# tensor4all/tensor4all-rs

Hardware: AMD Instinct MI355X
Metric: TCI2 full-sweep GF/s (d=30, chi=256 fp64) (higher is better)
Workload: dtype f64

## Files before the change

include/t4a_gpu.h:

```cpp
#ifndef T4A_GPU_H
#define T4A_GPU_H

#include <stddef.h>
#include <stdint.h>

#ifdef __cplusplus
extern "C" {
#endif
#if defined(__GNUC__)
#pragma GCC visibility push(default)
#endif

typedef int32_t t4a_gpu_status;
#define T4A_GPU_SUCCESS 0
#define T4A_GPU_NULL_POINTER (-1)
#define T4A_GPU_INVALID_ARGUMENT (-2)
#define T4A_GPU_BUFFER_TOO_SMALL (-5)
#define T4A_GPU_INTERNAL_ERROR (-6)
#define T4A_GPU_NOT_IMPLEMENTED (-7)
#define T4A_GPU_NAN_ENCOUNTERED (-8)
#define T4A_GPU_SINGULAR_MATRIX (-9)
#define T4A_GPU_NO_DEVICE (-10)
#define T4A_GPU_KERNEL_TIMEOUT (-11)
#define T4A_GPU_CALLBACK_ERROR (-12)
// ... 522 lines not shown
                                                     size_t* added);
t4a_gpu_status t4a_gpu_aci_problem_find_global_pivots(t4a_gpu_aci_problem* h, uint64_t seed, size_t* count, size_t* out);
t4a_gpu_status t4a_gpu_aci_problem_solution(t4a_gpu_aci_problem* h, t4a_gpu_tt** out);
t4a_gpu_status t4a_gpu_aci_problem_frame(t4a_gpu_aci_problem* h, int32_t right, size_t input, size_t site, size_t* rows,
                                         size_t* cols, double* out);
t4a_gpu_status t4a_gpu_aci_problem_errors(const t4a_gpu_aci_problem* h, double* pivot_errors, double* pivot_scales);

t4a_gpu_status t4a_gpu_treeaci_local_update_f64(size_t n_inputs, const size_t* bond_dims, const double* const* row_frames,
                                                const double* const* col_frames, size_t row_count, size_t col_count, int32_t op_kind,
                                                t4a_gpu_aci_op_fn op, void* user, size_t max_bond_dim, double tolerance,
                                                int32_t scale_tolerance, int32_t left_orthogonal, size_t* rank, size_t* row_indices,
                                                size_t* col_indices, double* pivot_errors, size_t* n_pivot_errors, double* left,
                                                double* right, double* sampled_scale, double* local_values);

t4a_gpu_status t4a_gpu_tci2_last_sweep_shapes(const t4a_gpu_tci2* h, size_t* out);
#define T4A_GPU_PROFILE_SLOTS 16
t4a_gpu_status t4a_gpu_tci2_profile_enable(t4a_gpu_tci2* h, int32_t enable);
t4a_gpu_status t4a_gpu_tci2_profile_reset(t4a_gpu_tci2* h);
t4a_gpu_status t4a_gpu_tci2_profile_get(const t4a_gpu_tci2* h, double* out );
t4a_gpu_status t4a_gpu_tci2_profile_variants(const t4a_gpu_tci2* h, double* out , size_t cap_rows, size_t* n_rows);

t4a_gpu_status t4a_gpu_tci2_chain_stats(const t4a_gpu_tci2* h, uint64_t* out );
t4a_gpu_status t4a_gpu_tci2_chain_stats_ext(const t4a_gpu_tci2* h, uint64_t* out );
t4a_gpu_status t4a_gpu_tci2_fill_stats(const t4a_gpu_tci2* h, uint64_t* out );
t4a_gpu_status t4a_gpu_tci2_rook_stats(const t4a_gpu_tci2* h, uint64_t* out );
t4a_gpu_status t4a_gpu_tci2_optimize_group(t4a_gpu_tci2* const* handles, size_t n_handles, const t4a_gpu_tci2_options* options,
                                           int32_t final_sweep1site);
t4a_gpu_status t4a_gpu_tci2_fill_site_tensors_group(t4a_gpu_tci2* const* handles, size_t n_handles);
t4a_gpu_status t4a_gpu_tci2_set_chain(t4a_gpu_tci2* h, int32_t enable, int32_t verify);
t4a_gpu_status t4a_gpu_tci2_set_callback_threads(t4a_gpu_tci2* h, size_t n_threads);
t4a_gpu_status t4a_gpu_tci2_small_stats(const t4a_gpu_tci2* h, uint64_t* out );

t4a_gpu_status t4a_gpu_fn_eval(int32_t fid, int32_t n_acc, const double* params, const uint64_t* weights,
                               const size_t* local_dims, size_t n_sites, const size_t* idx, size_t n_pts,
                               double* out);

#if defined(__GNUC__)
#pragma GCC visibility pop
#endif
#ifdef __cplusplus
}
#endif
#endif
```

tensor4all-rs_amd/csrc/capi.hip:

```cpp
#include "stdrng.hpp"
#include "smallrng.hpp"
#include <memory>
#include <initializer_list>
#include <mutex>

#include "patching.hpp"
#include "tci2.hpp"
#include "tree.hpp"
#include "quantics.hpp"
#include "tensorops.hpp"
#include "dense.hpp"
#include "aci.hpp"
#include "globalsearch.hpp"
#include "mpo.hpp"
#include "contraction.hpp"
#include "quanticstransform.hpp"
#include "tt_canonical.hpp"

struct t4a_gpu_tci2 {
    t4a::Tci2 impl;
    explicit t4a_gpu_tci2(const std::vector<size_t>& d) : impl(d) {}
};

struct t4a_gpu_treetci {
// ... 1065 lines not shown
            out[5 * i + 0] = (double)kv.first;
            for (int j = 0; j < 4; ++j) out[5 * i + 1 + j] = kv.second[j];
            ++i;
        }
    });
}


t4a_gpu_status t4a_gpu_tci2_chain_stats(const t4a_gpu_tci2* h, uint64_t* out)
{
    return guarded([&] {
        T4A_REQUIRE_PTR(h);
        T4A_REQUIRE_PTR(out);
        for (int k = 0; k < 5; ++k) out[k] = h->impl.chain_stats[k];
    });
}

t4a_gpu_status t4a_gpu_tci2_chain_stats_ext(const t4a_gpu_tci2* h, uint64_t* out)
{
    return guarded([&] {
        T4A_REQUIRE_PTR(h);
        T4A_REQUIRE_PTR(out);
        for (int k = 0; k < 4; ++k) out[k] = h->impl.chain_stats_ext[k];
    });
}

t4a_gpu_status t4a_gpu_tci2_rook_stats(const t4a_gpu_tci2* h, uint64_t* out)
{
    return guarded([&] {
        T4A_REQUIRE_PTR(h);
        T4A_REQUIRE_PTR(out);
        const RookWork& w = h->impl.rook_work();
        out[0] = w.n_device_searches;
        out[1] = w.n_device_visits;
        out[2] = w.n_host_searches;
        out[3] = w.n_host_syncs;
    });
}

t4a_gpu_status t4a_gpu_tci2_fill_stats(const t4a_gpu_tci2* h, uint64_t* out)
{
    return guarded([&] {
        T4A_REQUIRE_PTR(h);
        T4A_REQUIRE_PTR(out);
        for (int k = 0; k < 3; ++k) out[k] = h->impl.fill_stats()[k];
    });
// ... 2912 lines not shown
```

tensor4all-rs_amd/csrc/kernels.hpp:

```cpp
#pragma once

#include <hip/hip_runtime.h>

#include <cstddef>
#include <cstdint>

#include "../../include/t4a_testfunctions.h"

namespace t4a {

struct RrluWorkspace;

struct RrluPlan {
    int W = 1;
    int T = 256;
    int cpw = 0;
    int Mld = 0;
    size_t lds_bytes = 0;
};

RrluPlan rrlu_make_plan(int M, int N, int num_cus);

struct RrluArgs {
    const double* A;
// ... 239 lines not shown
    const int* prev_colperm;
    unsigned prev_token;
    unsigned long long* dbg;
    int defer_host_writes;
};
struct ChainWalkArgs {
    char* blocks;
    size_t block_bytes, off_piv, off_rp, off_cp, off_ts;
    double* pi;
    int n_bonds;
    int max_steps;
    double rel_tol, abs_tol;
    double* factors;
    size_t factors_stride;
    unsigned token_base;
    int timed;
    int lean_prep;
    unsigned long long* phase_ticks;
};
void chain_walk_launch(const ChainCommon& c, const FnDevice& fn, const ChainWalkArgs& w, int columns, hipStream_t stream);
void chain_indep_launch(const ChainCommon& c, int n_bonds, hipStream_t stream);
void chain_last_core_launch(const ChainCommon& c, const FnDevice& fn, double* core, int max_entries, hipStream_t stream);
void chain_prep_launch(const ChainCommon& c, const ChainPrepArgs& a, hipStream_t stream);
void chain_pi_launch(const ChainCommon& c, const FnDevice& fn, int b, int n_dep_ub, int n_ind_ub, double* out, hipStream_t stream);

constexpr int CHAIN_GROUP_MAX = 8;
struct ChainGroupSlot {
    ChainCommon c;
    FnDevice fn;
    double* pi;
};
struct ChainPrepGroupArgs {
    ChainPrepArgs a[CHAIN_GROUP_MAX];
};
void chain_indep_group_launch(const ChainGroupSlot* d_slots, int n_handles, int n_bonds, hipStream_t stream);
void chain_prep_group_launch(const ChainGroupSlot* d_slots, const ChainPrepGroupArgs& a, int n_handles, hipStream_t stream);
void chain_pi_group_launch(const ChainGroupSlot* d_slots, int n_handles, int b, int n_dep_ub, int n_ind_ub, hipStream_t stream);

struct GemmDesc {
    int m, n, k;
    const double* A; int lda; long long strideA; int transA;
    const double* B; int ldb; long long strideB; int transB;
    double* C; int ldc; long long strideC;
    double alpha, beta;
    int batch;
    int ksplit = 1;
    double* partial = nullptr;
};
void gemm_launch(const GemmDesc& d, hipStream_t stream);
inline GemmDesc gemm_desc(int m, int n, int k, const double* A, int lda, const double* B, int ldb, double* C, int ldc)
{
    GemmDesc g{};
    g.m = m;
    g.n = n;
    g.k = k;
    g.A = A;
    g.lda = lda;
    g.B = B;
    g.ldb = ldb;
// ... 227 lines not shown
```

tensor4all-rs_amd/csrc/kernels_chain.hip:

```cpp
#include "kernels.hpp"
#include "kernels_rrlu_w1_body.hpp"

namespace t4a {

namespace {

__device__ __forceinline__ const char* chain_kernarg_base()
{
#if defined(__HIP_DEVICE_COMPILE__)
    return (const char*)__builtin_amdgcn_kernarg_segment_ptr();
#else
    return nullptr;
#endif
}

constexpr int CHAIN_T = 1024;
constexpr int WALK_T = 1024;
constexpr int CHAIN_HASH = 4096;

__device__ __forceinline__ unsigned chain_hash(unsigned long long c)
{
    c ^= c >> 33;
    c *= 0xff51afd7ed558ccdull;
    c ^= c >> 29;
    return (unsigned)c & (CHAIN_HASH - 1);
}

__device__ __forceinline__ int block_scan_flag(bool flag, int* wave_sums, int* total)
{
    const int lane = threadIdx.x & 63, wave = threadIdx.x >> 6;
    const unsigned long long bal = __ballot(flag);
    const int before = __builtin_popcountll(bal & ((1ull << lane) - 1ull));
    __syncthreads();
    if (lane == 0) wave_sums[wave] = __builtin_popcountll(bal);
    __syncthreads();
    int base = 0, tot = 0;
    for (int w = 0; w < (int)blockDim.x / 64; ++w) {
        const int v = wave_sums[w];
        if (w < wave) base += v;
        tot += v;
    }
    *total = tot;
    return base + before;
}

template <bool PARENT_OUTER>
__device__ int build_side(const uint64_t* __restrict__ pcode, const uint64_t* __restrict__ pacc, int np, int d,
                          const uint64_t* __restrict__ w, int K, int total_w, int w_off, const uint64_t* __restrict__ ecode,
                          const uint64_t* __restrict__ eacc, int ne, uint64_t* __restrict__ ocode, uint64_t* __restrict__ oacc, int ocap,
// ... 240 lines not shown
        if (np >= 1 && np <= c.cap && ne <= c.cap)
            nd = build_side<false>(par_lds ? ws->par_code : c.J.code + (size_t)(b + 1) * cap, par_lds ? ws->par_acc : c.J.acc + (size_t)(b + 1) * cap * K, np, c.ldim[b + 1], c.w, K, c.total,
                                   c.woff[b + 1], xcode, xacc, ne, c.dep_code, c.dep_acc,
                                   c.dep_cap, s_srcpos, n_prev_dep, mapped ? c.rowmap : nullptr, hkeys, wave_sums);
        lda = n_prev_dep * c.ldim[b + 1] + ne;
    }
    stamp(5);
    if (tid == 0) {
        const int ni = c.ind_cnt[b];
        const bool ok = nd > 0 && ni > 0;
        const int M = c.forward ? nd : ni, N = c.forward ? ni : nd;
        dims[0] = ok ? M : 0;
        dims[1] = ok ? N : 0;
        dims[2] = ok ? 0 : 1;
        dims[3] = mapped ? lda : (ok ? nd : 0);
        if (hdims) {
            hdims[0] = ok ? M : 0;
            hdims[1] = ok ? N : 0;
            hdims[2] = ok ? 0 : 1;
        }
    }
}

__global__ void __launch_bounds__(CHAIN_T) chain_prep_kernel(ChainCommon c, ChainPrepArgs p)
{
    const unsigned long long t0 = p.dbg ? wall_clock64() : 0ull;
    chain_prep_body(c, p, p.dbg);
    if (p.dbg && threadIdx.x == 0) p.dbg[6] += wall_clock64() - t0;
}
__global__ void __launch_bounds__(CHAIN_T) chain_prep_group_kernel(const ChainGroupSlot* __restrict__ slots, ChainPrepGroupArgs g)
{
    const ChainPrepArgs* pa = reinterpret_cast<const ChainPrepArgs*>(chain_kernarg_base() + sizeof(const ChainGroupSlot*)) + blockIdx.x;
    (void)g;
    chain_prep_body(slots[blockIdx.x].c, *pa);
}

__device__ __forceinline__ void chain_pi_body(const ChainCommon& c, const FnDevice& fn, int b, double* __restrict__ out)
{
    const int* dm = c.dims + (size_t)b * 4;
    if (dm[2] != 0) return;
    const int K = fn.n_acc;
    const int nd = c.forward ? dm[0] : dm[1], ni = c.forward ? dm[1] : dm[0];
    const int i = blockIdx.x * blockDim.x + threadIdx.x;
    if (blockIdx.x * (int)blockDim.x >= nd) return;
    uint64_t racc[T4A_FN_MAX_ACC] = {0, 0, 0, 0};
    if (i < nd)
        for (int k = 0; k < K; ++k) racc[k] = c.dep_acc[(size_t)i * K + k];
    const uint64_t* ia = c.ind_acc + (size_t)b * c.ind_cap * K;
    for (int j = blockIdx.y; j < ni; j += gridDim.y) {
        if (i < nd) {
            uint64_t acc[T4A_FN_MAX_ACC] = {0, 0, 0, 0};
            for (int k = 0; k < K; ++k) acc[k] = racc[k] + ia[(size_t)j * K + k];
            out[(size_t)j * nd + i] = t4a_fn_value(fn.fid, acc, fn.params);
        }
    }
}
__global__ void __launch_bounds__(256) chain_pi_kernel(ChainCommon c, FnDevice fn, int b, double* __restrict__ out) { chain_pi_body(c, fn, b, out); }
// ... 8 lines not shown
{
    const int K = c.K;
    const size_t cap = (size_t)c.cap;
    const int gtid = (int)(blockIdx.x * blockDim.x + threadIdx.x), gsz = (int)(gridDim.x * blockDim.x);
    const int lane = (int)(threadIdx.x & 63), gwave = gtid >> 6, nwaves = gsz >> 6;
    for (int pf = gwave; pf < 2 * (nb + 1); pf += nwaves) {
        const int site = pf >> 1, fam = pf & 1;
        if ((fam == 0 && site == 0) || (fam == 1 && site == nb)) continue;
        const ChainTab& T = fam == 0 ? c.I : c.J;
        const ChainTab& Mr = fam == 0 ? c.mI : c.mJ;
        const int cnt = __hip_atomic_load(T.cnt + site, __ATOMIC_RELAXED, __HIP_MEMORY_SCOPE_AGENT);
        if (cnt < 0 || cnt > c.cap) continue;
        for (int e = lane; e < cnt * (1 + K); e += 64) {
            if (e < cnt) Mr.code[(size_t)site * cap + e] = T.code[(size_t)site * cap + e];
            else Mr.acc[(size_t)site * cap * K + (e - cnt)] = T.acc[(size_t)site * cap * K + (e - cnt)];
        }
        if (lane == 0) Mr.cnt[site] = cnt;
    }
    if (c.hdims)
        for (int e = gtid; e < nb * 4; e += gsz)
            if ((e & 3) != 3) c.hdims[e] = __hip_atomic_load(c.dims + e, __ATOMIC_RELAXED, __HIP_MEMORY_SCOPE_AGENT);
}

__global__ void __launch_bounds__(256) chain_last_core_kernel(ChainCommon c, FnDevice fn, double* __restrict__ core, int max_entries)
{
    const int site = c.n_sites - 1, K = c.K;
    const size_t cap = (size_t)c.cap;
    const int L = c.I.cnt[site], R = c.J.cnt[site], S = c.ldim[site], woff = c.woff[site];
    if (L < 1 || L > c.cap || R < 1 || R > c.cap || S < 1) return;
    const long long total = (long long)L * S * R;
    if (total > (long long)max_entries) return;
    for (long long e = (long long)blockIdx.x * blockDim.x + threadIdx.x; e < total; e += (long long)gridDim.x * blockDim.x) {
        const int l = (int)(e % L), s_ = (int)((e / L) % S), r = (int)(e / ((long long)L * S));
        uint64_t acc[T4A_FN_MAX_ACC] = {0, 0, 0, 0};
        for (int q = 0; q < K; ++q)
            acc[q] = c.I.acc[((size_t)site * cap + l) * K + q] + c.w[(size_t)q * c.total + woff + s_] + c.J.acc[((size_t)site * cap + r) * K + q];
        core[e] = t4a_fn_value(fn.fid, acc, fn.params);
    }
}

__device__ __forceinline__ void walk_phase_barrier(bool scalar_cache = true)
{
    if (scalar_cache) {
        __syncthreads();
        __builtin_amdgcn_s_dcache_inv();
        asm volatile("s_waitcnt lgkmcnt(0)" ::: "memory");
    } else {
        asm volatile("s_waitcnt lgkmcnt(0)\n\ts_barrier" ::: "memory");
    }
}
__device__ __forceinline__ int walk_div_small(int x, float rd) { return (int)(((float)x + 0.5f) * rd); }
__device__ __forceinline__ int walk_load_i32(const int* p) { return __hip_atomic_load(p, __ATOMIC_RELAXED, __HIP_MEMORY_SCOPE_AGENT); }

template <bool FORWARD>
__device__ __forceinline__ void walk_prep_wave0(const ChainCommon& c, WalkShared* ws, int b, int prev_b, unsigned prev_token, bool do_build, unsigned long long* dbg = nullptr)
{
    const unsigned long long dbg_t0 = dbg ? wall_clock64() : 0ull;
    const int lane = threadIdx.x & 63;
    const int K = c.K;
    const size_t cap = (size_t)c.cap;
    bool poison = false;
    int np = 0;
    if (prev_b >= 0) {
        const int pb = prev_b;
        const int pm = ws->dims[pb * 4], pn = ws->dims[pb * 4 + 1];
        const bool bad = ws->dims[pb * 4 + 2] != 0 || ws->prev_ires[1] != 0 || ws->prev_ires[3] != (int)prev_token || pm <= 0 || pn <= 0;
        const int r = ws->prev_ires[0];
        const int cnt = r > 0 ? r : 1;
        if (bad || cnt > c.cap || cnt > pm || cnt > pn || cnt > WALK_MAX_LIST) {
            poison = true;
        } else {
// ... 263 lines not shown
                    if (tid == 0) a.iresult[3] = (int)a.salt;
                }
            }
            if (tid == 0) {
                ws->prev_ires[0] = npiv >= 0 ? npiv : 0;
                ws->prev_ires[1] = npiv >= 0 ? 0 : 1;
                ws->prev_ires[2] = 0;
                ws->prev_ires[3] = npiv >= 0 ? (int)(w.token_base + (unsigned)k) : 0;
            }
        }
        walk_phase_barrier(!w.lean_prep);
        phase(2);
    }
    for (int e = tid; e < nb * 4; e += (int)blockDim.x) c.dims[e] = ws->dims[e];
    __threadfence();
    __syncthreads();
    chain_mirror_body(c, nb);
    if (w.phase_ticks && tid == 0) {
        for (int i = 0; i < 3; ++i) w.phase_ticks[i] = ph[i];
        w.phase_ticks[3] = wall_clock64() - ph_t0;
    }
}

template <int NC, bool FORWARD, bool FACTORS> void chain_walk_launch_one(const ChainCommon& c, const FnDevice& fn, const ChainWalkArgs& w, hipStream_t stream)
{
    constexpr size_t lds = walk_lds_bytes<NC, FACTORS>();
    static std::once_flag attr_once;
    std::call_once(attr_once, [] {
        (void)hipFuncSetAttribute(reinterpret_cast<const void*>(&chain_walk_kernel<NC, FORWARD, FACTORS>), hipFuncAttributeMaxDynamicSharedMemorySize, (int)lds);
    });
    hipLaunchKernelGGL((chain_walk_kernel<NC, FORWARD, FACTORS>), dim3(1), dim3(WALK_T), lds, stream, c, fn, w);
}

template <int NC> void chain_walk_launch_nc(const ChainCommon& c, const FnDevice& fn, const ChainWalkArgs& w, hipStream_t stream)
{
    if (w.factors) {
        if (c.forward) chain_walk_launch_one<NC, true, true>(c, fn, w, stream);
        else chain_walk_launch_one<NC, false, true>(c, fn, w, stream);
    } else {
        if (c.forward) chain_walk_launch_one<NC, true, false>(c, fn, w, stream);
        else chain_walk_launch_one<NC, false, false>(c, fn, w, stream);
    }
}

}

void chain_indep_launch(const ChainCommon& c, int n_bonds, hipStream_t stream)
{
    hipLaunchKernelGGL(chain_indep_kernel, dim3(n_bonds), dim3(CHAIN_T), 0, stream, c);
}

void chain_prep_launch(const ChainCommon& c, const ChainPrepArgs& a, hipStream_t stream)
{
    hipLaunchKernelGGL(chain_prep_kernel, dim3(1), dim3(CHAIN_T), 0, stream, c, a);
}

void chain_pi_launch(const ChainCommon& c, const FnDevice& fn, int b, int n_dep_ub, int n_ind_ub, double* out, hipStream_t stream)
{
    if (n_dep_ub <= 0 || n_ind_ub <= 0) return;
    const int gy = n_ind_ub < 2048 ? n_ind_ub : 2048;
    hipLaunchKernelGGL(chain_pi_kernel, dim3((n_dep_ub + 255) / 256, gy), dim3(256), 0, stream, c, fn, b, out);
}

void chain_indep_group_launch(const ChainGroupSlot* d_slots, int n_handles, int n_bonds, hipStream_t stream)
{
    hipLaunchKernelGGL(chain_indep_group_kernel, dim3(n_bonds, n_handles), dim3(CHAIN_T), 0, stream, d_slots);
}

void chain_prep_group_launch(const ChainGroupSlot* d_slots, const ChainPrepGroupArgs& a, int n_handles, hipStream_t stream)
{
    hipLaunchKernelGGL(chain_prep_group_kernel, dim3(n_handles), dim3(CHAIN_T), 0, stream, d_slots, a);
}

void chain_pi_group_launch(const ChainGroupSlot* d_slots, int n_handles, int b, int n_dep_ub, int n_ind_ub, hipStream_t stream)
{
    if (n_dep_ub <= 0 || n_ind_ub <= 0 || n_handles <= 0) return;
    const int gy = n_ind_ub < 2048 ? n_ind_ub : 2048;
    hipLaunchKernelGGL(chain_pi_group_kernel, dim3((n_dep_ub + 255) / 256, gy, n_handles), dim3(256), 0, stream, d_slots, b);
}

void chain_walk_launch(const ChainCommon& c, const FnDevice& fn, const ChainWalkArgs& w, int columns, hipStream_t stream)
{
    if (columns <= 8) chain_walk_launch_nc<8>(c, fn, w, stream);
    else if (columns <= 16) chain_walk_launch_nc<16>(c, fn, w, stream);
    else chain_walk_launch_nc<32>(c, fn, w, stream);
}

void chain_last_core_launch(const ChainCommon& c, const FnDevice& fn, double* core, int max_entries, hipStream_t stream)
{
    const int blocks = max_entries > 256 * 64 ? 64 : (max_entries + 255) / 256;
    hipLaunchKernelGGL(chain_last_core_kernel, dim3(blocks > 0 ? blocks : 1), dim3(256), 0, stream, c, fn, core, max_entries);
}

}
// ... 1 lines not shown
```

tensor4all-rs_amd/csrc/tci2.hpp:

```cpp
#pragma once

#include <cstring>
#include <memory>
#include <vector>

#include "engine.hpp"
#include "fnsource.hpp"
#include "matrix_source.hpp"
#include "stdrng.hpp"
#include "pishard.hpp"
#include "rook.hpp"
#include "tt.hpp"

namespace t4a {

struct TCI2Options {
    double tolerance = 1e-8;
    size_t max_iter = 20;
    size_t max_bond_dim = 0;
    int pivot_search = 0;
    bool normalize_error = true;
    size_t verbosity = 0;
    size_t max_nglobal_pivot = 5;
    size_t nsearch = 5;
// ... 99 lines not shown
    bool small_engine_run(OptRun& r);
    void opt_begin(OptRun& r);
    void opt_issue_pending_fill(OptRun& r);
    bool opt_iter_start(OptRun& r, bool defer_launch = false);
    void opt_iter_finish(OptRun& r);
    void opt_end(OptRun& r);
    void sweep2site(bool forward, const TCI2Options& options);
    void sweep1site(bool forward, double rel_tol, double abs_tol, size_t max_bond_dim, bool update_tensors);
    void fill_site_tensors();
    void fill_wait();
    void export_site_tensors_async(double* d_dst, size_t stride, hipStream_t consumer);
    void export_site_shard_async(double* d_dst, size_t stride, hipStream_t consumer);
    void import_site_shard_async(const double* d_src, size_t stride, size_t per_rank, hipStream_t producer);
    void make_canonical(double rel_tol, double abs_tol, size_t max_bond_dim);
    void invalidate_site_tensors();
    void flush_pivot_errors() { pivot_errors.clear(); }
    void mark_sets_changed()
    {
        chain_.tables_valid = false;
        chain_.digits_stale = false;
    }
    std::array<uint64_t, 5> chain_stats{{0, 0, 0, 0, 0}};
    std::array<uint64_t, 4> chain_stats_ext{{0, 0, 0, 0}};
    const uint64_t* fill_stats() const { return fill_.stats; }
    const RookWork& rook_work() const { return rook_work_; }
    bool chain_enabled = true;
    bool chain_verify = false;
    bool chain_event_timing = false;

    std::vector<double> evaluate(const uint32_t* idx, size_t n_pts);
    double sum();
    std::vector<double> site_tensor_host(size_t site, size_t dims3[3]);

    void assign_from_tensor_train(const TensorTrain& tt, const FromTensorTrainOptions& options);

    size_t n_;
    std::vector<size_t> local_dims;
    std::vector<IndexSet> i_set, j_set;
    struct HistEntry {
        std::vector<IndexSet> is, js;
        bool digits_valid = true;
        std::vector<uint64_t> code;
        size_t cap = 0;
        uint64_t serial = 0;
    };
    std::vector<HistEntry> history;
// ... 118 lines not shown
        DevBuf<int> dims;
        PinBuf<int> hdims;
        bool inflight = false;
        bool forward = true;
        bool in_optimize = false;
        long ext_idx = -1;
        size_t chi = 0;
        std::vector<size_t> order;
        std::vector<RrluRoute> plans;
        std::vector<unsigned> tokens;
        bool one_site = false;
        bool one_factors = false;
        double abs_tol = 0.0;
        DevBuf<double> factors, urows;
        size_t factors_stride = 0;
        bool cores_batched = false;
        bool last_core_launched = false, last_core_ok = false;
        DevBuf<unsigned long long> walk_dbg;
        bool walked = false;
        bool prep_dbg = false;
        unsigned walk_token = 1;
        RrluBlock proto;
        bool timed = false, timed_events = false;
        std::vector<hipEvent_t> t0, t1;
        bool prepared = false;
        ChainCommon common;
        std::vector<size_t> dep_ub, ind_ub;
        bool use_extras = false;
        size_t ind_cap = 0, cap_side = 0;
        double tol = 0.0;
        hipStream_t wait_stream = nullptr;
        int group_role = 0;
        hipEvent_t group_ev = nullptr;
        DevBuf<ChainGroupSlot> gslots;
        PinBuf<ChainGroupSlot> hgslots;
    } chain_;
    bool chain_usable(const TCI2Options& options) const;
    ChainTab chain_tab(int family) const;
    ChainTab chain_mirror(int which, int family) const;
    void chain_layout(size_t cap);
    void chain_upload_current();
    void chain_upload_hist(HistEntry& e, int slot);
    uint64_t code_of(const uint32_t* v, size_t first_site, size_t width, bool prefix) const;
    void decode_set(IndexSet& s, const uint64_t* codes, size_t first_site, bool prefix) const;
    void hist_digits(HistEntry& e);
    bool chain_enqueue(bool forward, const TCI2Options& options, long ext_idx, bool in_optimize, bool launch = true);
// ... 27 lines not shown
```

tensor4all-rs_amd/csrc/tci2_chain.hip:

```cpp
#include "tci2.hpp"

#include <algorithm>
#include <atomic>
#include <chrono>
#include <cmath>
#include <cstdlib>

namespace t4a {

namespace {
size_t round_up_sz(size_t v, size_t m) { return (v + m - 1) / m * m; }
std::atomic<int> g_chains_inflight{0};
}
thread_local double g_chain_wait_seconds = 0.0;

bool Tci2::chain_usable(const TCI2Options& options) const
{
    static const bool off = std::getenv("T4A_NO_CHAIN") != nullptr;
    if (off || !chain_enabled || !fn_.builtin() || options.pivot_search != 0) return false;
    long double space = 1.0L;
    for (size_t d : local_dims) space *= (long double)d;
    if (space >= 9.0e18L) return false;
    for (size_t p = 0; p < n_; ++p) {
        if (i_set[p].count == 0 || j_set[p].count == 0) return false;
// ... 469 lines not shown
            chain_walk_launch(c, fn_.dev, w, (int)walk_cols, st);
            ++chain_stats_ext[0];
        }
        static const bool want_prep_dbg = std::getenv("T4A_PREP_DEBUG") != nullptr;
        unsigned long long* prep_dbg = nullptr;
        if (want_prep_dbg && !walk) {
            chain_.walk_dbg.reserve(8);
            T4A_HIP(hipMemsetAsync(chain_.walk_dbg.get(), 0, 8 * sizeof(unsigned long long), st));
            prep_dbg = chain_.walk_dbg.get();
            chain_.prep_dbg = true;
        }
        bool spec_pending = false;
        for (size_t k = 0; !walk && k < nb; ++k) {
            const size_t b = order[k];
            const RrluRoute& pl = plans[b];
            const bool fused = pl.fused;
            const bool spec_here = spec_pending && !fused;
            const RrluBlock blk = block_of(b);
            ChainPrepArgs pa;
            std::memset(&pa, 0, sizeof(pa));
            pa.b = (int)b;
            pa.do_build = 1;
            pa.dbg = prep_dbg;
            pa.defer_host_writes = 0;
            pa.with_rowmap = spec_here ? 1 : 0;
            pa.prev_b = -1;
            if (k > 0) {
                const size_t pb = order[k - 1];
                const RrluBlock pblk = block_of(pb);
                pa.prev_b = (int)pb;
                pa.prev_iresult = pblk.iresult();
                pa.prev_rowperm = pblk.row_perm();
                pa.prev_colperm = pblk.col_perm();
                pa.prev_token = tokens[pb];
            }
            chain_prep_launch(c, pa, st);
            if (!fused && !spec_here) chain_pi_launch(c, fn_.dev, (int)b, (int)dep_ub[b], (int)ind_ub[b], chain_.pi.get(), st);
            XcdSpecArgs sp;
            std::memset(&sp, 0, sizeof(sp));
            spec_pending = false;
            if (solo && k + 1 < nb && pl.on_xcd()) {
                const size_t nx = order[k + 1];
                if (!plans[nx].fused) {
                    const size_t site = forward ? nx : nx + 1;
                    const ChainTab& H = forward ? c.HI : c.HJ;
                    const size_t hsite = forward ? nx + 1 : nx;
                    sp.out = chain_.spec[(k + 1) & 1].get();
// ... 8 lines not shown
                    sp.d = (int)local_dims[site];
                    sp.fn = fn_.dev;
                    spec_pending = true;
                }
            }
            FusedPi fp;
            fp.fn = fn_.dev;
            fp.d_rowacc = c.dep_acc;
            fp.d_colacc = c.ind_acc + b * ind_cap * K;
            fp.host_resident = false;
            const double* A = fused ? nullptr : (spec_here ? chain_.spec[k & 1].get() : chain_.pi.get());
            if (timed_events) T4A_HIP(hipEventRecord(chain_.t0[b], st));
            tokens[b] = eng.chain_rrlu(pl, forward, A, spec_here ? c.rowmap : nullptr, fused ? &fp : nullptr, c.dims + b * 4, chi, chain_.tol,
                                       chain_.one_site ? chain_.abs_tol : 0.0, blk, spec_pending ? &sp : nullptr,
                                       chain_.factors_stride ? chain_.factors.get() + b * chain_.factors_stride : nullptr, chain_.urows.get());
            if (timed_events) T4A_HIP(hipEventRecord(chain_.t1[b], st));
        }
        if (!walk) {
            const size_t pb = order[nb - 1];
            const RrluBlock pblk = block_of(pb);
            ChainPrepArgs pa;
            std::memset(&pa, 0, sizeof(pa));
            pa.do_build = 0;
            pa.defer_host_writes = 0;
            pa.prev_b = (int)pb;
            pa.prev_iresult = pblk.iresult();
            pa.prev_rowperm = pblk.row_perm();
            pa.prev_colperm = pblk.col_perm();
            pa.prev_token = tokens[pb];
            chain_prep_launch(c, pa, st);
        }
        chain_.cores_batched = false;
        if (chain_.one_site && chain_.factors_stride && forward && nb <= (size_t)LUCI_LEFT_CORES_MAX_JOBS) {
            LeftCoreJobs jobs;
            std::memset(&jobs, 0, sizeof(jobs));
            size_t max_rows = 1;
            for (size_t b = 0; b < nb; ++b) {
                const RrluBlock blk = block_of(b);
                const size_t rub = std::max<size_t>(std::min({dep_ub[b], ind_ub[b], chi}), 1);
                DevCore& core = cores[b];
                core.buf.reserve(std::max<size_t>(dep_ub[b] * rub, 1));
                LeftCoreJob& j = jobs.j[b];
                j.lu = chain_.factors.get() + b * chain_.factors_stride;
                j.dims = c.dims + b * 4;
                j.iresult = blk.iresult();
                j.row_perm = blk.row_perm();
                j.core = core.buf.get();
                j.S = (int)local_dims[b];
                j.token = tokens[b];
                max_rows = std::max(max_rows, dep_ub[b]);
            }
            luci_left_cores_batched_launch(jobs, (int)nb, (int)max_rows, st);
            chain_.cores_batched = true;
// ... 89 lines not shown
        auto block_of = [&](Tci2* h, size_t b) {
            RrluBlock k = h->chain_.proto;
            k.dev = h->chain_.blocks.get() + b * k.bytes;
            return k;
        };
        auto prev_of = [&](Tci2* h, size_t pb, ChainPrepArgs& pa) {
            const RrluBlock pblk = block_of(h, pb);
            pa.prev_b = (int)pb;
            pa.prev_iresult = pblk.iresult();
            pa.prev_rowperm = pblk.row_perm();
            pa.prev_colperm = pblk.col_perm();
            pa.prev_token = h->chain_.tokens[pb];
        };
        chain_indep_group_launch(d_slots, (int)nh, (int)nb, st);
        const std::vector<size_t>& order = lead->chain_.order;
        for (size_t k = 0; k < nb; ++k) {
            const size_t b = order[k];
            ChainPrepGroupArgs pg;
            std::memset(&pg, 0, sizeof(pg));
            for (size_t i = 0; i < nh; ++i) {
                ChainPrepArgs& pa = pg.a[i];
                pa.b = (int)b;
                pa.do_build = 1;
                pa.prev_b = -1;
                if (k > 0) prev_of(hs[i], order[k - 1], pa);
            }
            chain_prep_group_launch(d_slots, pg, (int)nh, st);
            chain_pi_group_launch(d_slots, (int)nh, (int)b, gplans[b].kM, gplans[b].kN, st);
            RrluXcdGroupArgs ga;
            std::memset(&ga, 0, sizeof(ga));
            for (int x = 0; x < 8; ++x) ga.p[x].xcc = -1;
            for (size_t i = 0; i < nh; ++i) {
                Tci2* h = hs[i];
                h->chain_.tokens[b] = h->eng.chain_group_args(gplans[b], forward, h->chain_.pi.get(), h->chain_.common.dims + b * 4, h->chain_.chi,
                                                              h->chain_.tol, 0.0, block_of(h, b), (int)i, &ga.p[i], st);
            }
            gplans[b].launch_group(ga, !forward, st);
        }
        {
            ChainPrepGroupArgs pg;
            std::memset(&pg, 0, sizeof(pg));
            for (size_t i = 0; i < nh; ++i) prev_of(hs[i], order[nb - 1], pg.a[i]);
            chain_prep_group_launch(d_slots, pg, (int)nh, st);
        }
        for (Tci2* h : hs)
            T4A_HIP(hipMemcpyAsync(h->chain_.hblocks.get(), h->chain_.blocks.get(), nb * h->chain_.proto.bytes, hipMemcpyDeviceToHost, st));
        T4A_HIP(hipGetLastError());
    } catch (...) {
        (void)hipStreamSynchronize(st);
        if (locked) lead->eng.chain_end();
        for (size_t i = 0; i < nh; ++i) {
            if (counted[i]) g_chains_inflight.fetch_sub(1);
            hs[i]->chain_.prepared = false;
            hs[i]->chain_.tables_valid = false;
            hs[i]->chain_.snap_serial[0] = hs[i]->chain_.snap_serial[1] = ~0ull;
        }
        throw;
    }
    for (Tci2* h : hs) {
        h->chain_.plans = gplans;
        h->chain_.inflight = true;
        h->chain_.wait_stream = st;
        h->chain_.group_role = h == lead ? 1 : 2;
    }
}

// ... 69 lines not shown
        if (hi[1] != 0 || hi[3] != (int)chain_.tokens[b]) {
            failed_k = (long)k;
            failed_timeout = hi[1] != 2;
            break;
        }
        if (hi[2] != 0) {
            failed_k = (long)k;
            break;
        }
    }
    if (failed_k >= 0) {
        static const bool dbg = std::getenv("T4A_CHAIN_DEBUG") != nullptr;
        if (dbg) {
            const size_t b = chain_.order[(size_t)failed_k];
            const int* hd = chain_.hdims.get() + b * 4;
            const int* hi = reinterpret_cast<const int*>(chain_.hblocks.get() + b * proto.bytes + 16);
            const RrluRoute& pl = chain_.plans[b];
            std::fprintf(stderr, "[t4a chain] bond %zu (k = %ld of %zu, %s) did not complete: dims %d x %d poisoned %d lda %d | npiv %d flag %d nan %d token %d (want %u) | plan kind %d %d x %d wg %d RPT %d CPT %d W %d\n",
                         b, failed_k, nb, forward ? "forward" : "backward", hd[0], hd[1], hd[2], hd[3], hi[0], hi[1], hi[2], hi[3], chain_.tokens[b], (int)pl.kind, pl.kM, pl.kN,
                         pl.xcd.wg, pl.xcd.RPT, pl.xcd.CPT, pl.xcd.W);
        }
    }
    const size_t done = failed_k < 0 ? nb : (size_t)failed_k;
    for (size_t k = 0; k < done; ++k) {
        const size_t b = chain_.order[k];
        const int* hd = chain_.hdims.get() + b * 4;
        const char* hb = chain_.hblocks.get() + b * proto.bytes;
        const int* hi = reinterpret_cast<const int*>(hb + 16);
        const size_t M = (size_t)hd[0], N = (size_t)hd[1];
        const int rank = hi[0];
        double last_error, abs_max;
        std::memcpy(&last_error, hb, sizeof(double));
        std::memcpy(&abs_max, hb + 8, sizeof(double));
        const size_t cnt = (size_t)(rank > 0 ? rank : 1);
        if ((size_t)ni.cnt[b + 1] != cnt || (size_t)nj.cnt[b] != cnt)
            throw Error(T4A_GPU_INTERNAL_ERROR, "bond chain: gathered pivot count of bond " + std::to_string(b) + " disagrees with its rank");
        i_set[b + 1].count = cnt;
        j_set[b].count = cnt;
        i_set[b + 1].d.clear();
        j_set[b].d.clear();
        {
            float ms = 0.f;
            if (chain_.timed) {
                unsigned long long ts[2];
                std::memcpy(ts, hb + proto.off_ts, sizeof(ts));
                ms = ts[1] > ts[0] ? (float)((double)(ts[1] - ts[0]) * 1e-5) : 0.f;
                if (chain_.timed_events) T4A_HIP(hipEventElapsedTime(&ms, chain_.t0[b], chain_.t1[b]));
                eng.prof.v[0] += ms;
                eng.prof.v[1] += 1.0;
            }
            eng.rrlu_account(chain_.plans[b], !forward, (int)M, (int)N, rank, chain_.timed, ms, chain_.chi > 0 && (size_t)rank == chain_.chi);
            eng.prof.v[11] += (double)M * (double)N;
        }
        if (abs_max > max_sample_value) max_sample_value = abs_max;
        bond_errors[b] = last_error;
        if (chain_.one_site) {
            std::vector<double> pe((size_t)rank + 1);
            const double* pv = reinterpret_cast<const double*>(hb + proto.off_piv);
            for (int q = 0; q < rank; ++q) pe[(size_t)q] = std::sqrt(pv[q] * pv[q]);
            pe[(size_t)rank] = last_error;
            update_pivot_errors(pe);
        } else {
            last_sweep_shapes[b] = {M, N, (size_t)rank};
        }
    }
    if (done > 0) {
        const ChainTab oi = chain_mirror(chain_.mcur, 0), oj = chain_mirror(chain_.mcur, 1);
        std::vector<char> wi(n_, 0), wj(n_, 0);
        for (size_t k = 0; k < done; ++k) {
// ... 130 lines not shown
```

tensor4all-rs_amd/python/t4a_amd/__init__.py:

```python
import ctypes
import os

import numpy as np

from .functions import (FnSpec, quantics_trig_exp, quantics_osc2d, lorentz, linear_sum,
                        FN_MAX_PARAMS)

_HERE = os.path.dirname(os.path.abspath(__file__))
LIB_PATH = os.environ.get("T4A_GPU_LIB") or os.path.normpath(os.path.join(_HERE, "..", "..", "lib", "libt4a_gpu.so"))

if not os.path.exists(LIB_PATH):
    raise ImportError(f"{LIB_PATH} not found: build it with `python tensor4all-rs_amd/build.py` "
                      "(the MI355X backend has no CPU fallback)")

_lib = ctypes.CDLL(LIB_PATH)

c_size_t = ctypes.c_size_t
c_double = ctypes.c_double
c_int32 = ctypes.c_int32
c_void_p = ctypes.c_void_p

SUCCESS = 0
NULL_POINTER = -1
INVALID_ARGUMENT = -2
# ... 737 lines not shown
        _check(_lib.t4a_gpu_tci2_small_stats(self._h, out))
        return {"completed": int(out[0]), "iterations": int(out[1]), "handed_back": int(out[2]), "not_eligible": int(out[3]),
                "device_us": (out[4] / 100.0, out[5] / 100.0, out[6] / 100.0), "reason": int(out[7]),
                "phase_cycles": dict(zip(("lists", "evaluation", "pivot_steps", "gather", "factors", "fill", "snapshots", "rest"), (int(out[8 + k]) for k in range(8))))}

    def rook_stats(self):
        out = (ctypes.c_uint64 * 4)()
        _check(_lib.t4a_gpu_tci2_rook_stats(self._h, out))
        return {"device_searches": int(out[0]), "device_visits": int(out[1]), "host_searches": int(out[2]), "host_syncs": int(out[3])}

    def fill_stats(self):
        out = (ctypes.c_uint64 * 3)()
        _check(_lib.t4a_gpu_tci2_fill_stats(self._h, out))
        return {"fills": int(out[0]), "graph_replays": int(out[1]), "graph_captures": int(out[2])}

    def chain_stats(self):
        out = np.zeros(5, dtype=np.uint64)
        _check(_lib.t4a_gpu_tci2_chain_stats(self._h, _p(out)))
        ext = np.zeros(4, dtype=np.uint64)
        _check(_lib.t4a_gpu_tci2_chain_stats_ext(self._h, _p(ext)))
        return dict(half_sweeps=int(out[0]), bonds=int(out[1]), fell_back=int(out[2]), not_eligible=int(out[3]),
                    group_half_sweeps=int(out[4]), walked_sweeps=int(ext[0]), one_site_sweeps=int(ext[1]),
                    one_site_not_eligible=int(ext[2]), one_site_fell_back=int(ext[3]))


def optimize_group(tcis, options, final_sweep1site=True):
    o = options.to_c()
    arr = (c_void_p * len(tcis))(*[t._h for t in tcis])
    _check(_lib.t4a_gpu_tci2_optimize_group(arr, c_size_t(len(tcis)), ctypes.byref(o), c_int32(1 if final_sweep1site else 0)))


def fill_site_tensors_group(tcis):
    arr = (c_void_p * len(tcis))(*[t._h for t in tcis])
    _check(_lib.t4a_gpu_tci2_fill_site_tensors_group(arr, c_size_t(len(tcis))))


def crossinterpolate2(f, local_dims, initial_pivots, options):
    options.to_c()
    tci = TensorCI2(local_dims)
    tci.set_function(f)
    tci.crossinterpolate2(initial_pivots, options)
    return tci


def svd_backend(a):
    a = _f(a)
# ... 1212 lines not shown
```

Baseline: 329.6.

## Add lean LDS-staged chain prep kernel and defer host-mirror writes to batched mirror pass

```diff
diff --git a/include/t4a_gpu.h b/include/t4a_gpu.h
--- a/include/t4a_gpu.h
+++ b/include/t4a_gpu.h
@@ -568,6 +568,7 @@
 
 t4a_gpu_status t4a_gpu_tci2_chain_stats(const t4a_gpu_tci2* h, uint64_t* out );
 t4a_gpu_status t4a_gpu_tci2_chain_stats_ext(const t4a_gpu_tci2* h, uint64_t* out );
+t4a_gpu_status t4a_gpu_tci2_chain_handover(const t4a_gpu_tci2* h, size_t* count, double* interval_us, int32_t* steps);
 t4a_gpu_status t4a_gpu_tci2_fill_stats(const t4a_gpu_tci2* h, uint64_t* out );
 t4a_gpu_status t4a_gpu_tci2_rook_stats(const t4a_gpu_tci2* h, uint64_t* out );
 t4a_gpu_status t4a_gpu_tci2_optimize_group(t4a_gpu_tci2* const* handles, size_t n_handles, const t4a_gpu_tci2_options* options,
diff --git a/tensor4all-rs_amd/csrc/capi.hip b/tensor4all-rs_amd/csrc/capi.hip
--- a/tensor4all-rs_amd/csrc/capi.hip
+++ b/tensor4all-rs_amd/csrc/capi.hip
@@ -1111,6 +1111,21 @@
         T4A_REQUIRE_PTR(h);
         T4A_REQUIRE_PTR(out);
         for (int k = 0; k < 4; ++k) out[k] = h->impl.chain_stats_ext[k];
+    });
+}
+
+t4a_gpu_status t4a_gpu_tci2_chain_handover(const t4a_gpu_tci2* h, size_t* count, double* interval_us, int32_t* steps)
+{
+    return guarded([&] {
+        T4A_REQUIRE_PTR(h);
+        T4A_REQUIRE_PTR(count);
+        const auto& v = h->impl.chain_handover();
+        *count = v.size();
+        if (interval_us && steps)
+            for (size_t k = 0; k < v.size(); ++k) {
+                interval_us[k] = v[k][0];
+                steps[k] = (int32_t)v[k][1];
+            }
     });
 }
 
diff --git a/tensor4all-rs_amd/csrc/kernels.hpp b/tensor4all-rs_amd/csrc/kernels.hpp
--- a/tensor4all-rs_amd/csrc/kernels.hpp
+++ b/tensor4all-rs_amd/csrc/kernels.hpp
@@ -285,6 +285,7 @@
 void chain_indep_launch(const ChainCommon& c, int n_bonds, hipStream_t stream);
 void chain_last_core_launch(const ChainCommon& c, const FnDevice& fn, double* core, int max_entries, hipStream_t stream);
 void chain_prep_launch(const ChainCommon& c, const ChainPrepArgs& a, hipStream_t stream);
+void chain_mirror_launch(const ChainCommon& c, int n_bonds, hipStream_t stream);
 void chain_pi_launch(const ChainCommon& c, const FnDevice& fn, int b, int n_dep_ub, int n_ind_ub, double* out, hipStream_t stream);
 
 constexpr int CHAIN_GROUP_MAX = 8;
@@ -298,6 +299,7 @@
 };
 void chain_indep_group_launch(const ChainGroupSlot* d_slots, int n_handles, int n_bonds, hipStream_t stream);
 void chain_prep_group_launch(const ChainGroupSlot* d_slots, const ChainPrepGroupArgs& a, int n_handles, hipStream_t stream);
+void chain_mirror_group_launch(const ChainGroupSlot* d_slots, int n_handles, int n_bonds, hipStream_t stream);
 void chain_pi_group_launch(const ChainGroupSlot* d_slots, int n_handles, int b, int n_dep_ub, int n_ind_ub, hipStream_t stream);
 
 struct GemmDesc {
diff --git a/tensor4all-rs_amd/csrc/kernels_chain.hip b/tensor4all-rs_amd/csrc/kernels_chain.hip
--- a/tensor4all-rs_amd/csrc/kernels_chain.hip
+++ b/tensor4all-rs_amd/csrc/kernels_chain.hip
@@ -1,5 +1,6 @@
 #include "kernels.hpp"
 #include "kernels_rrlu_w1_body.hpp"
+#include <atomic>
 
 namespace t4a {
 
@@ -25,6 +26,11 @@
     c ^= c >> 29;
     return (unsigned)c & (CHAIN_HASH - 1);
 }
+
+__device__ __forceinline__ void chain_lds_barrier() { asm volatile("s_waitcnt lgkmcnt(0)\n\ts_barrier" ::: "memory"); }
+
+__device__ __forceinline__ void chain_touch(uint64_t v) { asm volatile("" ::"v"(v) : "memory"); }
+__device__ __forceinline__ void chain_touch(int v) { asm volatile("" ::"v"(v) : "memory"); }
 
 __device__ __forceinline__ int block_scan_flag(bool flag, int* wave_sums, int* total)
 {
@@ -311,17 +317,262 @@
     }
 }
 
+constexpr int PREP_MAX_W = 2 * CHAIN_T;
+static_assert(CHAIN_MAX_SET <= CHAIN_T, "the lean preparation keeps one table entry (parent, extra, permutation entry) per thread");
+static_assert(CHAIN_T / 64 <= 64, "the wave counts of the compaction are combined by the lanes of one wave");
+struct PrepShared {
+    unsigned long long hkeys[CHAIN_HASH];
+    uint64_t par_code[CHAIN_MAX_SET], par_acc[CHAIN_MAX_SET * T4A_FN_MAX_ACC];
+    uint64_t w[PREP_MAX_W];
+    int srcpos[CHAIN_MAX_SET];
+    int wave_sums[CHAIN_T / 64];
+};
+
+__device__ __forceinline__ void chain_prep_lean_body(const ChainCommon& c, const ChainPrepArgs& p, PrepShared* sh, unsigned long long* dbg)
+{
+    unsigned long long dbg_last = dbg ? wall_clock64() : 0ull;
+    auto stamp = [&](int slot) {
+        if (dbg) {
+            const unsigned long long now = wall_clock64();
+            if (threadIdx.x == 0) dbg[slot] += now - dbg_last;
+            dbg_last = now;
+        }
+    };
+    const int tid = threadIdx.x, lane = tid & 63, wave = tid >> 6;
+    const int K = c.K, capi = c.cap;
+    const size_t cap = (size_t)c.cap;
+    const bool fwd = c.forward != 0, have_prev = p.prev_b >= 0, build = p.do_build != 0;
+    const bool extras = build && c.use_extras != 0;
+    const int pb = have_prev ? p.prev_b : 0, b = build ? p.b : 0;
+    if (capi < 1 || capi > CHAIN_MAX_SET || K < 1 || K > T4A_FN_MAX_ACC) return;
+    const int tcl = tid < capi ? tid : capi - 1;
+    if (extras) {
+#pragma unroll
+        for (int e = 0; e < CHAIN_HASH / CHAIN_T; ++e) sh->hkeys[tid + e * CHAIN_T] = 0ull;
+    }
+
+    const int* const pd = c.dims + (size_t)pb * 4;
+    const int* const irp = have_prev ? p.prev_iresult : c.dims;
+    const int rlim_ = fwd ? c.dep_cap : c.ind_cap, clim_ = fwd ? c.ind_cap : c.dep_cap;
+    const int rlim = have_prev && rlim_ > 1 ? rlim_ : 1, clim = have_prev && clim_ > 1 ? clim_ : 1;
+    const int* const rpp = have_prev ? p.prev_rowperm : c.dims;
+    const int* const cpp = have_prev ? p.prev_colperm : c.dims;
+    const int site = fwd ? b : b + 1;
+    const int hsite = fwd ? b + 1 : b;
+    const ChainTab& H = fwd ? c.HI : c.HJ;
+    const ChainTab& PT = fwd ? c.I : c.J;
+    const int nw = K * c.total;
+    const bool w_lds = nw >= 1 && nw <= PREP_MAX_W;
+    const int nwc = nw < 1 ? 1 : (nw > PREP_MAX_W ? PREP_MAX_W : nw);
+    const int pd0 = pd[0], pd1 = pd[1], pd2 = pd[2];
+    const int ir0 = irp[0], ir1 = irp[1], ir3 = irp[3];
+    const int rp = rpp[tcl < rlim ? tcl : rlim - 1], cp = cpp[tcl < clim ? tcl : clim - 1];
+    const int ni = c.ind_cnt[b], d = c.ldim[site], woff = c.woff[site];
+    const int ne_raw = H.cnt[hsite], np0 = PT.cnt[site];
+    const uint64_t w0 = c.w[tid < nwc ? tid : nwc - 1], w1 = c.w[tid + CHAIN_T < nwc ? tid + CHAIN_T : nwc - 1];
+    const uint64_t xc = H.code[(size_t)hsite * cap + tcl];
+    uint64_t xa[T4A_FN_MAX_ACC], pa[T4A_FN_MAX_ACC];
+#pragma unroll
+    for (int q = 0; q < T4A_FN_MAX_ACC; ++q) xa[q] = H.acc[((size_t)hsite * cap + tcl) * K + (q < K ? q : K - 1)];
+    uint64_t pc = PT.code[(size_t)site * cap + tcl];
+#pragma unroll
+    for (int q = 0; q < T4A_FN_MAX_ACC; ++q) pa[q] = PT.acc[((size_t)site * cap + tcl) * K + (q < K ? q : K - 1)];
+
+    const bool bad = (pd2 != 0) | (ir1 != 0) | (ir3 != (int)p.prev_token) | (pd0 <= 0) | (pd1 <= 0);
+    const int r = ir0;
+    const int cnt = r > 0 ? r : 1;
+    const bool poison = have_prev & (bad | (cnt > capi) | (cnt > pd0) | (cnt > pd1));
+    const int n_prev_dep = (have_prev & !poison) ? (fwd ? pd0 : pd1) : 0;
+
+    const bool gather = have_prev && !poison;
+    chain_touch(rp), chain_touch(cp);
+    const bool mine = gather && tid < cnt;
+    uint64_t rc = 0, cc = 0, ra[T4A_FN_MAX_ACC] = {0, 0, 0, 0}, ca[T4A_FN_MAX_ACC] = {0, 0, 0, 0};
+    int src = 0;
+    if (gather) {
+        const uint64_t* const pind_code = c.ind_code + (size_t)pb * c.ind_cap;
+        const uint64_t* const pind_acc = c.ind_acc + (size_t)pb * c.ind_cap * K;
+        const uint64_t* rcode = fwd ? c.dep_code : pind_code;
+        const uint64_t* racc = fwd ? c.dep_acc : pind_acc;
+        const uint64_t* ccode = fwd ? pind_code : c.dep_code;
+        const uint64_t* cacc = fwd ? pind_acc : c.dep_acc;
+        const int ri = (mine && r > 0) ? rp : 0, ci = (mine && r > 0) ? cp : 0;
+        rc = rcode[ri];
+        cc = ccode[ci];
+#pragma unroll
+        for (int q = 0; q < T4A_FN_MAX_ACC; ++q) {
+            ra[q] = racc[(size_t)ri * K + (q < K ? q : K - 1)];
+            ca[q] = cacc[(size_t)ci * K + (q < K ? q : K - 1)];
+        }
+        src = fwd ? ri : ci;
+    }
+    const unsigned long long xkey = (unsigned long long)(xc / (uint64_t)(d > 0 ? d : 1)) + 1ull;
+    chain_touch(rc), chain_touch(cc), chain_touch(xc), chain_touch(pc), chain_touch(w0), chain_touch(w1);
+#pragma unroll
+    for (int q = 0; q < T4A_FN_MAX_ACC; ++q) chain_touch(ra[q]), chain_touch(ca[q]), chain_touch(xa[q]), chain_touch(pa[q]);
+    if (gather) {
+        pc = fwd ? rc : cc;
+#pragma unroll
+        for (int q = 0; q < T4A_FN_MAX_ACC; ++q) pa[q] = fwd ? ra[q] : ca[q];
+    }
+    const int np = have_prev ? cnt : np0;
+    const int ne = extras ? ne_raw : 0;
+    const bool sides_ok = np >= 1 && np <= capi && ne <= capi;
+    if (build && !poison) {
+        if (sides_ok && tid < np) {
+            sh->par_code[tid] = pc;
+#pragma unroll
+            for (int q = 0; q < T4A_FN_MAX_ACC; ++q)
+                if (q < K) sh->par_acc[(size_t)tid * K + q] = pa[q];
+            sh->srcpos[tid] = src;
+        }
+        if (w_lds) {
+            if (tid < nw) sh->w[tid] = w0;
+            if (tid + CHAIN_T < nw) sh->w[tid + CHAIN_T] = w1;
+        }
+    }
+    if (mine) {
+        const size_t oi = (size_t)(pb + 1) * cap + tid, oj = (size_t)pb * cap + tid;
+        c.I.code[oi] = rc;
+        c.J.code[oj] = cc;
+#pragma unroll
+        for (int q = 0; q < T4A_FN_MAX_ACC; ++q)
+            if (q < K) {
+                c.I.acc[oi * K + q] = ra[q];
+                c.J.acc[oj * K + q] = ca[q];
+            }
+        if (!p.defer_host_writes) {
+            c.mI.code[oi] = rc;
+            c.mJ.code[oj] = cc;
+#pragma unroll
+            for (int q = 0; q < T4A_FN_MAX_ACC; ++q)
+                if (q < K) {
+                    c.mI.acc[oi * K + q] = ra[q];
+                    c.mJ.acc[oj * K + q] = ca[q];
+                }
+        }
+    }
+    if (gather && tid == 0) {
+        c.I.cnt[pb + 1] = cnt;
+        c.J.cnt[pb] = cnt;
+        if (!p.defer_host_writes) {
+            c.mI.cnt[pb + 1] = cnt;
+            c.mJ.cnt[pb] = cnt;
+        }
+    }
+    stamp(4);
+    if (!build) return;
+    int* dims = c.dims + (size_t)b * 4;
+    int* hdims = (c.hdims && !p.defer_host_writes) ? c.hdims + (size_t)b * 4 : nullptr;
+    if (poison) {
+        if (tid == 0) {
+            dims[0] = dims[1] = dims[3] = 0;
+            dims[2] = 1;
+            if (hdims) {
+                hdims[0] = hdims[1] = 0;
+                hdims[2] = 1;
+            }
+        }
+        return;
+    }
+
+    const bool mapped = have_prev && p.with_rowmap;
+    chain_lds_barrier();
+    int nd = -1;
+    const int m0 = np * d;
+    if (sides_ok && m0 <= c.dep_cap) {
+        auto kron = [&](const uint64_t* __restrict__ wsrc) {
+            for (int idx = tid; idx < m0; idx += CHAIN_T) {
+                const int i = fwd ? idx / d : idx % np;
+                const int s = fwd ? idx % d : idx / np;
+                c.dep_code[idx] = (uint64_t)s + (uint64_t)d * sh->par_code[i];
+                for (int k = 0; k < K; ++k) c.dep_acc[(size_t)idx * K + k] = sh->par_acc[(size_t)i * K + k] + wsrc[(size_t)k * c.total + woff + s];
+                if (mapped) c.rowmap[idx] = sh->srcpos[i] * d + s;
+            }
+        };
+        if (w_lds) kron(sh->w);
+        else kron(c.w);
+        if (ne <= 0) {
+            nd = m0;
+        } else {
+            if (tid < np) {
+                const unsigned long long key = (unsigned long long)pc + 1ull;
+                unsigned h = chain_hash(key);
+                for (;;) {
+                    const unsigned long long old = atomicCAS(&sh->hkeys[h], 0ull, key);
+                    if (old == 0ull || old == key) break;
+                    h = (h + 1) & (CHAIN_HASH - 1);
+                }
+            }
+            chain_lds_barrier();
+            bool keep = false;
+            if (tid < ne) {
+                unsigned h = chain_hash(xkey);
+                keep = true;
+                for (;;) {
+                    const unsigned long long v = sh->hkeys[h];
+                    if (v == 0ull) break;
+                    if (v == xkey) {
+                        keep = false;
+                        break;
+                    }
+                    h = (h + 1) & (CHAIN_HASH - 1);
+                }
+            }
+            const unsigned long long bal = __ballot(keep);
+            if (lane == 0) sh->wave_sums[wave] = __builtin_popcountll(bal);
+            chain_lds_barrier();
+            int v = lane < CHAIN_T / 64 ? sh->wave_sums[lane] : 0;
+            int vb = lane < wave ? v : 0;
+#pragma unroll
+            for (int off = 32; off >= 1; off >>= 1) {
+                v += __shfl_xor(v, off);
+                vb += __shfl_xor(vb, off);
+            }
+            const int tot = v;
+            if (m0 + tot <= c.dep_cap) {
+                if (keep) {
+                    const int o = m0 + vb + __builtin_popcountll(bal & ((1ull << lane) - 1ull));
+                    c.dep_code[o] = xc;
+#pragma unroll
+                    for (int k = 0; k < T4A_FN_MAX_ACC; ++k)
+                        if (k < K) c.dep_acc[(size_t)o * K + k] = xa[k];
+                    if (mapped) c.rowmap[o] = n_prev_dep * d + tid;
+                }
+                nd = m0 + tot;
+            }
+        }
+    }
+    stamp(5);
+    if (tid == 0) {
+        const int lda = n_prev_dep * d + ne;
+        const bool ok = nd > 0 && ni > 0;
+        const int M = fwd ? nd : ni, N = fwd ? ni : nd;
+        dims[0] = ok ? M : 0;
+        dims[1] = ok ? N : 0;
+        dims[2] = ok ? 0 : 1;
+        dims[3] = mapped ? lda : (ok ? nd : 0);
+        if (hdims) {
+            hdims[0] = ok ? M : 0;
+            hdims[1] = ok ? N : 0;
+            hdims[2] = ok ? 0 : 1;
+        }
+    }
+}
+
 __global__ void __launch_bounds__(CHAIN_T) chain_prep_kernel(ChainCommon c, ChainPrepArgs p)
 {
+    extern __shared__ __attribute__((aligned(16))) char prep_lds[];
     const unsigned long long t0 = p.dbg ? wall_clock64() : 0ull;
-    chain_prep_body(c, p, p.dbg);
+    chain_prep_lean_body(c, p, reinterpret_cast<PrepShared*>(prep_lds), p.dbg);
     if (p.dbg && threadIdx.x == 0) p.dbg[6] += wall_clock64() - t0;
 }
 __global__ void __launch_bounds__(CHAIN_T) chain_prep_group_kernel(const ChainGroupSlot* __restrict__ slots, ChainPrepGroupArgs g)
 {
+    extern __shared__ __attribute__((aligned(16))) char prep_group_lds[];
     const ChainPrepArgs* pa = reinterpret_cast<const ChainPrepArgs*>(chain_kernarg_base() + sizeof(const ChainGroupSlot*)) + blockIdx.x;
     (void)g;
-    chain_prep_body(slots[blockIdx.x].c, *pa);
+    chain_prep_lean_body(slots[blockIdx.x].c, *pa, reinterpret_cast<PrepShared*>(prep_group_lds), nullptr);
 }
 
 __device__ __forceinline__ void chain_pi_body(const ChainCommon& c, const FnDevice& fn, int b, double* __restrict__ out)
@@ -376,6 +627,9 @@
             if ((e & 3) != 3) c.hdims[e] = __hip_atomic_load(c.dims + e, __ATOMIC_RELAXED, __HIP_MEMORY_SCOPE_AGENT);
 }
 
+__global__ void __launch_bounds__(256) chain_mirror_kernel(ChainCommon c, int nb) { chain_mirror_body(c, nb); }
+__global__ void __launch_bounds__(256) chain_mirror_group_kernel(const ChainGroupSlot* __restrict__ slots, int nb) { chain_mirror_body(slots[blockIdx.y].c, nb); }
+
 __global__ void __launch_bounds__(256) chain_last_core_kernel(ChainCommon c, FnDevice fn, double* __restrict__ core, int max_entries)
 {
     const int site = c.n_sites - 1, K = c.K;
@@ -400,7 +654,7 @@
         __builtin_amdgcn_s_dcache_inv();
         asm volatile("s_waitcnt lgkmcnt(0)" ::: "memory");
     } else {
-        asm volatile("s_waitcnt lgkmcnt(0)\n\ts_barrier" ::: "memory");
+        chain_lds_barrier();
     }
 }
 __device__ __forceinline__ int walk_div_small(int x, float rd) { return (int)(((float)x + 0.5f) * rd); }
@@ -710,6 +964,16 @@
     }
 }
 
+void prep_lds_attribute(const void* kernel, std::atomic<unsigned long long>& done)
+{
+    int dev = 0;
+    (void)hipGetDevice(&dev);
+    const unsigned long long bit = 1ull << (dev & 63);
+    if (done.load(std::memory_order_relaxed) & bit) return;
+    (void)hipFuncSetAttribute(kernel, hipFuncAttributeMaxDynamicSharedMemorySize, (int)sizeof(PrepShared));
+    done.fetch_or(bit, std::memory_order_relaxed);
+}
+
 template <int NC, bool FORWARD, bool FACTORS> void chain_walk_launch_one(const ChainCommon& c, const FnDevice& fn, const ChainWalkArgs& w, hipStream_t stream)
 {
     constexpr size_t lds = walk_lds_bytes<NC, FACTORS>();
@@ -740,7 +1004,15 @@
 
 void chain_prep_launch(const ChainCommon& c, const ChainPrepArgs& a, hipStream_t stream)
 {
-    hipLaunchKernelGGL(chain_prep_kernel, dim3(1), dim3(CHAIN_T), 0, stream, c, a);
+    static std::atomic<unsigned long long> attr_done{0ull};
+    prep_lds_attribute(reinterpret_cast<const void*>(&chain_prep_kernel), attr_done);
+    hipLaunchKernelGGL(chain_prep_kernel, dim3(1), dim3(CHAIN_T), sizeof(PrepShared), stream, c, a);
+}
+
+void chain_mirror_launch(const ChainCommon& c, int n_bonds, hipStream_t stream)
+{
+    const int waves = 2 * (n_bonds + 1);
+    hipLaunchKernelGGL(chain_mirror_kernel, dim3((waves + 3) / 4), dim3(256), 0, stream, c, n_bonds);
 }
 
 void chain_pi_launch(const ChainCommon& c, const FnDevice& fn, int b, int n_dep_ub, int n_ind_ub, double* out, hipStream_t stream)
@@ -757,7 +1029,15 @@
 
 void chain_prep_group_launch(const ChainGroupSlot* d_slots, const ChainPrepGroupArgs& a, int n_handles, hipStream_t stream)
 {
-    hipLaunchKernelGGL(chain_prep_group_kernel, dim3(n_handles), dim3(CHAIN_T), 0, stream, d_slots, a);
+    static std::atomic<unsigned long long> attr_done{0ull};
+    prep_lds_attribute(reinterpret_cast<const void*>(&chain_prep_group_kernel), attr_done);
+    hipLaunchKernelGGL(chain_prep_group_kernel, dim3(n_handles), dim3(CHAIN_T), sizeof(PrepShared), stream, d_slots, a);
+}
+
+void chain_mirror_group_launch(const ChainGroupSlot* d_slots, int n_handles, int n_bonds, hipStream_t stream)
+{
+    const int waves = 2 * (n_bonds + 1);
+    hipLaunchKernelGGL(chain_mirror_group_kernel, dim3((waves + 3) / 4, n_handles), dim3(256), 0, stream, d_slots, n_bonds);
 }
 
 void chain_pi_group_launch(const ChainGroupSlot* d_slots, int n_handles, int b, int n_dep_ub, int n_ind_ub, hipStream_t stream)
diff --git a/tensor4all-rs_amd/csrc/tci2.hpp b/tensor4all-rs_amd/csrc/tci2.hpp
--- a/tensor4all-rs_amd/csrc/tci2.hpp
+++ b/tensor4all-rs_amd/csrc/tci2.hpp
@@ -145,6 +145,7 @@
     }
     std::array<uint64_t, 5> chain_stats{{0, 0, 0, 0, 0}};
     std::array<uint64_t, 4> chain_stats_ext{{0, 0, 0, 0}};
+    const std::vector<std::array<double, 2>>& chain_handover() const { return chain_.handover; }
     const uint64_t* fill_stats() const { return fill_.stats; }
     const RookWork& rook_work() const { return rook_work_; }
     bool chain_enabled = true;
@@ -309,6 +310,7 @@
         unsigned walk_token = 1;
         RrluBlock proto;
         bool timed = false, timed_events = false;
+        std::vector<std::array<double, 2>> handover;
         std::vector<hipEvent_t> t0, t1;
         bool prepared = false;
         ChainCommon common;
diff --git a/tensor4all-rs_amd/csrc/tci2_chain.hip b/tensor4all-rs_amd/csrc/tci2_chain.hip
--- a/tensor4all-rs_amd/csrc/tci2_chain.hip
+++ b/tensor4all-rs_amd/csrc/tci2_chain.hip
@@ -515,7 +515,7 @@
             pa.b = (int)b;
             pa.do_build = 1;
             pa.dbg = prep_dbg;
-            pa.defer_host_writes = 0;
+            pa.defer_host_writes = 1;
             pa.with_rowmap = spec_here ? 1 : 0;
             pa.prev_b = -1;
             if (k > 0) {
@@ -570,13 +570,14 @@
             ChainPrepArgs pa;
             std::memset(&pa, 0, sizeof(pa));
             pa.do_build = 0;
-            pa.defer_host_writes = 0;
+            pa.defer_host_writes = 1;
             pa.prev_b = (int)pb;
             pa.prev_iresult = pblk.iresult();
             pa.prev_rowperm = pblk.row_perm();
             pa.prev_colperm = pblk.col_perm();
             pa.prev_token = tokens[pb];
             chain_prep_launch(c, pa, st);
+            chain_mirror_launch(c, (int)nb, st);
         }
         chain_.cores_batched = false;
         if (chain_.one_site && chain_.factors_stride && forward && nb <= (size_t)LUCI_LEFT_CORES_MAX_JOBS) {
@@ -712,6 +713,7 @@
                 ChainPrepArgs& pa = pg.a[i];
                 pa.b = (int)b;
                 pa.do_build = 1;
+                pa.defer_host_writes = 1;
                 pa.prev_b = -1;
                 if (k > 0) prev_of(hs[i], order[k - 1], pa);
             }
@@ -730,8 +732,12 @@
         {
             ChainPrepGroupArgs pg;
             std::memset(&pg, 0, sizeof(pg));
-            for (size_t i = 0; i < nh; ++i) prev_of(hs[i], order[nb - 1], pg.a[i]);
+            for (size_t i = 0; i < nh; ++i) {
+                prev_of(hs[i], order[nb - 1], pg.a[i]);
+                pg.a[i].defer_host_writes = 1;
+            }
             chain_prep_group_launch(d_slots, pg, (int)nh, st);
+            chain_mirror_group_launch(d_slots, (int)nh, (int)nb, st);
         }
         for (Tci2* h : hs)
             T4A_HIP(hipMemcpyAsync(h->chain_.hblocks.get(), h->chain_.blocks.get(), nb * h->chain_.proto.bytes, hipMemcpyDeviceToHost, st));
@@ -847,6 +853,8 @@
         }
     }
     const size_t done = failed_k < 0 ? nb : (size_t)failed_k;
+    unsigned long long prev_end = 0ull;
+    if (chain_.timed) chain_.handover.clear();
     for (size_t k = 0; k < done; ++k) {
         const size_t b = chain_.order[k];
         const int* hd = chain_.hdims.get() + b * 4;
@@ -870,6 +878,8 @@
                 unsigned long long ts[2];
                 std::memcpy(ts, hb + proto.off_ts, sizeof(ts));
                 ms = ts[1] > ts[0] ? (float)((double)(ts[1] - ts[0]) * 1e-5) : 0.f;
+                chain_.handover.push_back({k > 0 && prev_end != 0ull ? (double)((long long)(ts[0] - prev_end)) * 0.01 : -1.0, (double)rank});
+                prev_end = ts[1];
                 if (chain_.timed_events) T4A_HIP(hipEventElapsedTime(&ms, chain_.t0[b], chain_.t1[b]));
                 eng.prof.v[0] += ms;
                 eng.prof.v[1] += 1.0;
diff --git a/tensor4all-rs_amd/python/t4a_amd/__init__.py b/tensor4all-rs_amd/python/t4a_amd/__init__.py
--- a/tensor4all-rs_amd/python/t4a_amd/__init__.py
+++ b/tensor4all-rs_amd/python/t4a_amd/__init__.py
@@ -783,6 +783,14 @@
         return dict(half_sweeps=int(out[0]), bonds=int(out[1]), fell_back=int(out[2]), not_eligible=int(out[3]),
                     group_half_sweeps=int(out[4]), walked_sweeps=int(ext[0]), one_site_sweeps=int(ext[1]),
                     one_site_not_eligible=int(ext[2]), one_site_fell_back=int(ext[3]))
+
+    def chain_handover(self):
+        n = c_size_t(0)
+        _check(_lib.t4a_gpu_tci2_chain_handover(self._h, ctypes.byref(n), None, None))
+        us = np.zeros(max(n.value, 1), dtype=np.float64)
+        steps = np.zeros(max(n.value, 1), dtype=np.int32)
+        _check(_lib.t4a_gpu_tci2_chain_handover(self._h, ctypes.byref(n), _p(us), _p(steps)))
+        return us[: n.value], steps[: n.value]
 
 
 def optimize_group(tcis, options, final_sweep1site=True):
```

After: 331.6 (median of 4 runs). About the same (+0.6%).
